# awkrail/svpc

Measured on AMD Instinct MI355X. Metric: train steps/sec (vivt, batch=16, clip_seq=12), higher is better.
Workload: dtype bf16x3; 1 GPU; MODEL_TYPE=vivt train step: N=16 videos/GPU x S=12 clips x Lv=100 frames x F=3072, Lt=22, D=768, H=12, L=6 (enc+step-enc+dec), V=951, A=384, E=10; dropout .1/.1/.4; fwd+bwd+allreduce+clip+BertAdam; mode=bf16x3, global_batch=16, parallelism=dp1, launch=hipGraph replay, gpus_requested=1

## Files before the change

### include/svpc_hip.h

```cpp
#ifndef SVPC_HIP_H
#define SVPC_HIP_H
#include <stddef.h>
#ifdef __cplusplus
extern "C" {
#endif

typedef struct ihipStream_t* svpc_stream_t;
typedef unsigned long long svpc_u64;

#define SVPC_ACT_NONE 0
#define SVPC_ACT_RELU 1
#define SVPC_ACT_GELU 2
#define SVPC_ACT_SIGMOID 3

const char* svpc_last_error(void);
int svpc_abi_version(void);

int svpc_ln_fwd(const float* x, const int* src_rows, const float* res, const float* gamma, const float* beta, float* y,
                float* mean, float* rstd, int R, int D, float eps, float p_pre, unsigned site_pre, float p_post,
                unsigned site_post, const svpc_u64* seed, const float* add1, int mod1, const float* add2, const int* idx2,
                svpc_stream_t stream);
int svpc_ln_fwd_t(const void* x, int x_dt, const int* src_rows, const void* res, const float* gamma, const float* beta, void* y,
                  int y_dt, float* mean, float* rstd, int R, int D, float eps, float p_pre, unsigned site_pre, float p_post,
                  unsigned site_post, const svpc_u64* seed, const float* add1, int mod1, const float* add2, const int* idx2,
// ... 85 lines not shown
} svpc_wgrad_problem;
int svpc_gemm_group_wgrad_max(void);
int svpc_gemm_group_wgrad_bf16_p8_ok(const void* problems, int n);
int svpc_gemm_group_wgrad_bf16_p8(const void* problems, int n, float* workspace, size_t workspace_bytes, svpc_stream_t stream);
int svpc_gemm_group_wgrad_bf16(const svpc_wgrad_problem* problems, int n, svpc_stream_t stream);
int svpc_gemm_group_wgrad_bf16_ws(const svpc_wgrad_problem* problems, int n, float* workspace, size_t workspace_bytes,
                                  svpc_stream_t stream);
int svpc_gemm_group_wgrad(const svpc_wgrad_problem* problems, int n, svpc_stream_t stream);
int svpc_act_bwd(const float* dy, const float* aux, float* dz, size_t n, int act, float p, unsigned site, const svpc_u64* seed,
                 svpc_stream_t stream);

int svpc_act_bwd_t(const void* dy, const void* aux, void* dz, int dt, size_t n, int act, float p, unsigned site, const svpc_u64* seed,
                   svpc_stream_t stream);

int svpc_attn_fwd(const float* Q, int ldq, const float* K, int ldk, const float* V, int ldv, float* O, int ldo, float* LSE,
                  const int* seq, int n_seq, int H, int dh, int max_q, int max_k, const float* key_mask, int causal, float scale,
                  float p_drop, unsigned site, const svpc_u64* seed, svpc_stream_t stream);
int svpc_attn_q1_fwd(const float* Q, int ldq, const float* K, int ldk, const float* V, int ldv, float* O, int ldo, float* LSE,
                     const int* seq, int n_seq, int H, int dh, int max_k, const float* key_mask, float scale, svpc_stream_t stream);
int svpc_attn_q1_ln_supported(int D, int dh, int n_keys, int ldq, int ldkv, int ldnew, int ldx, int ldo);
int svpc_attn_q1_ln_fwd(const float* Q, int ldq, float* K, float* V, int ldkv, int k_stride, int n_keys, const float* newK, const float* newV,
                        int ldnew, const float* X, int ldx, const float* gamma, const float* beta, float eps, float* O, int ldo, int T, int D,
                        int dh, float scale, svpc_stream_t stream);
int svpc_attn_q1_ln_idx_fwd(const float* Q, int ldq, float* K, float* V, int ldkv, int k_stride, int n_keys, const int* key_rows, int ld_rows,
                            int q_group, const float* newK, const float* newV, int ldnew, const float* X, int ldx, const float* gamma,
                            const float* beta, float eps, float* O, int ldo, int T, int D, int dh, float scale, svpc_stream_t stream);
int svpc_attn_bwd(const float* Q, int ldq, const float* K, int ldk, const float* V, int ldv, const float* O, int ldo,
                  const float* LSE, const float* dO, int lddo, float* dQ, int lddq, float* dK, int lddk, float* dV, int lddv,
                  float* delta, const int* seq, int n_seq, int H, int dh, int max_q, int max_k, const float* key_mask, int causal,
                  float scale, float p_drop, unsigned site, const svpc_u64* seed, svpc_stream_t stream);

int svpc_attn_mfma_supported(int dh, int max_q, int max_k, int ldq, int ldk, int ldv, int dt );
int svpc_attn_mfma_fwd(const float* Q, int ldq, const float* K, int ldk, const float* V, int ldv, float* O, int ldo, float* LSE,
                       const int* seq, int n_seq, int H, int dh, int max_q, int max_k, const float* key_mask, int causal,
                       float scale, float p_drop, unsigned site, const svpc_u64* seed, svpc_stream_t stream);
int svpc_attn_mfma_bwd(const float* Q, int ldq, const float* K, int ldk, const float* V, int ldv, const float* O, int ldo,
                       const float* LSE, const float* dO, int lddo, float* dQ, int lddq, float* dK, int lddk, float* dV, int lddv,
                       const int* seq, int n_seq, int H, int dh, int max_q, int max_k, const float* key_mask, int causal, float scale,
                       float p_drop, unsigned site, const svpc_u64* seed, svpc_stream_t stream);

int svpc_attn_mfma_fwd_t(const void* Q, int ldq, const void* K, int ldk, const void* V, int ldv, void* O, int ldo, int dt, float* LSE,
                         const int* seq, int n_seq, int H, int dh, int max_q, int max_k, const float* key_mask, int causal,
                         float scale, float p_drop, unsigned site, const svpc_u64* seed, svpc_stream_t stream);
int svpc_attn_stream_x3_fwd(const void* Q, int ldq, int q_lo, const void* K, int ldk, int k_lo, const void* V, int ldv, int v_lo, void* O,
                            int ldo, int o_lo, float* LSE, const int* seq, int n_seq, int H, int dh, int max_q, int max_k,
                            const float* key_mask, float scale, float p_drop, unsigned site, const svpc_u64* seed, svpc_stream_t stream);
int svpc_attn_q1s_supported(int dh, int max_k, int ldq, int ldk, int ldv, int k_lo, int v_lo);
int svpc_attn_q1s_fwd(const float* Q, int ldq, const void* K, int ldk, int k_lo, const void* V, int ldv, int v_lo, float* O, int ldo, float* LSE,
                      const int* seq, int n_seq, int H, int dh, int max_k, const float* key_mask, float scale, float p_drop, unsigned site,
                      const svpc_u64* seed, svpc_stream_t stream);
int svpc_attn_q1s_bwd(const float* Q, int ldq, const void* K, int ldk, int k_lo, const void* V, int ldv, int v_lo, const float* dO, int lddo,
                      float* dQ, int lddq, void* dK, int lddk, void* dV, int lddv, const int* seq, int n_seq, int H, int dh, int max_k,
                      const float* key_mask, float scale, float p_drop, unsigned site, const svpc_u64* seed, svpc_stream_t stream);
int svpc_attn_x3_fwd(const void* Q, int ldq, int q_lo, const void* K, int ldk, int k_lo, const void* V, int ldv, int v_lo, void* O, int ldo,
                     int o_lo, float* LSE, const int* seq, int n_seq, int H, int dh, int max_q, int max_k, const float* key_mask, int causal,
                     float scale, float p_drop, unsigned site, const svpc_u64* seed, svpc_stream_t stream);
int svpc_attn_pipe_enable(int on);
int svpc_attn_pipe_debug(int bits, void* buf);
int svpc_attn_mfma_bwd_t(const void* Q, int ldq, const void* K, int ldk, const void* V, int ldv, const void* O, int ldo, int dt,
                         const float* LSE, const void* dO, int lddo, void* dQ, int lddq, void* dK, int lddk, void* dV, int lddv,
                         const int* seq, int n_seq, int H, int dh, int max_q, int max_k, const float* key_mask, int causal, float scale,
                         float p_drop, unsigned site, const svpc_u64* seed, svpc_stream_t stream);

int svpc_sim_recur_fwd(const float* q, const float* c, const float* w4f, const float* E0, const int* step_off, const int* step_len,
                       const int* ent_off, const int* ent_len, int n_videos, int e_max, int D, float* e_out, float* ebar,
                       float* eall, svpc_stream_t stream);
int svpc_sim_recur_bwd(const float* q, const float* c, const float* w4f, const float* E0, const int* step_off, const int* step_len,
                       const int* ent_off, const int* ent_len, int n_videos, int e_max, int D, const float* e_out,
                       const float* ebar, const float* eall, const float* de, const float* debar, const float* deall, float* dq,
                       float* dc, float* dw4f, float* dE0, svpc_stream_t stream);

int svpc_sim_heads_groups(int T);
int svpc_sim_heads_fwd(const float* hh, const float* fb, const float* W3, const float* b3, const float* W4, const float* b4, float* c, float* w,
                       int T, int D, int Wd, svpc_stream_t stream);
int svpc_sim_heads_bwd(const float* hh, const float* fb, const float* W3, const float* W4, const float* c, const float* dc, const float* dw,
                       float* dhh, float* dfb, float* part3, float* part4, int T, int D, int Wd, svpc_stream_t stream);

int svpc_cross_attn_ln_supported(int D, int H, int lt, int nm);
int svpc_cross_attn_ln_fwd(const void* q, int q_dt, int ldq, int loq, const void* x1, int x_dt, int ldx, int lox, const void* k, const void* v,
                           int kv_dt, int ld_kv, int lokv, const float* gamma, const float* beta, float eps, void* y, int y_dt, int ldy, int loy,
                           float* probs, float* mean, float* rstd, int T, int lt, int nm, int D, int H, float scale, float p_drop, unsigned site,
                           const svpc_u64* seed, svpc_stream_t stream);
int svpc_cross_attn_ln_bwd(const void* q, int q_dt, int ldq, int loq, const void* x1, int x_dt, int ldx, int lox, const void* k, const void* v,
                           int kv_dt, int ld_kv, int lokv, const float* gamma, const float* probs, const float* mean, const float* rstd,
                           const void* dy, int dy_dt, int lddy, void* dq, void* dres, int dg_dt, int lddg, void* dk, void* dv, int dkv_dt,
                           int ld_dkv, float* part_ln, int T, int lt, int nm, int D, int H, float scale, float p_drop, unsigned site,
                           const svpc_u64* seed, svpc_stream_t stream);
int svpc_cross_attn_ln_fwd_r(const void* q, int q_dt, int ldq, int loq, const void* x1, int x_dt, int ldx, int lox, const void* k, const void* v,
                             int kv_dt, int ld_kv, int lokv, const float* gamma, const float* beta, float eps, void* y, int y_dt, int ldy, int loy,
                             float* probs, float* mean, float* rstd, int T, int lt, int nm, int D, int H, float scale, float p_drop, unsigned site,
                             const svpc_u64* seed, const int* row_off, const int* row_len, svpc_stream_t stream);
int svpc_cross_attn_ln_bwd_r(const void* q, int q_dt, int ldq, int loq, const void* x1, int x_dt, int ldx, int lox, const void* k, const void* v,
                             int kv_dt, int ld_kv, int lokv, const float* gamma, const float* probs, const float* mean, const float* rstd,
                             const void* dy, int dy_dt, int lddy, void* dq, void* dres, int dg_dt, int lddg, void* dk, void* dv, int dkv_dt,
                             int ld_dkv, float* part_ln, int T, int lt, int nm, int D, int H, float scale, float p_drop, unsigned site,
                             const svpc_u64* seed, const int* row_off, const int* row_len, svpc_stream_t stream);

int svpc_ptr_attn_fwd(const float* dec, const float* proj, const float* bank, const int* step_ne, float* pi, float* att, int T,
                      int lt, int e_max, int D, svpc_stream_t stream);
int svpc_ptr_attn_pgen_fwd(const float* dec, const float* proj, const float* bank, const int* step_ne, float* pi, float* att,
                           const float* pgen_w, const float* pgen_b, float* pgen, int T, int lt, int e_max, int D, svpc_stream_t stream);
int svpc_ptr_attn_bwd(const float* dec, const float* proj, const float* bank, const int* step_ne, const float* pi, const float* dpi,
                      const float* datt, float* ddec, float* dproj, float* dbank, int T, int lt, int e_max, int D,
                      svpc_stream_t stream);
int svpc_ptr_attn_gate_fwd(const float* dec, const float* proj, const float* bank, const int* step_ne, float* pi, const float* pgen_w,
                           const float* pgen_b, float* pgen, int T, int lt, int e_max, int D, svpc_stream_t stream);
// ... 223 lines not shown
```

### svpc_amd/grad_tail.py

```python
from __future__ import annotations

import ctypes
import os

import torch

from . import _lib

USE_GROUPED_WGRAD = os.environ.get("SVPC_NO_GROUPED_WGRAD", "") == ""
GROUP_BF16 = os.environ.get("SVPC_NO_GROUP_BF16", "") == ""
GROUP_FLUSH_AT = int(os.environ.get("SVPC_GROUP_FLUSH_AT", "16"))
GROUP_MAX_TILES = int(os.environ.get("SVPC_GROUP_MAX_TILES", "1200"))
COLSUM_FLUSH_AT = 48

_WQ16 = []
_WQ = []
_CQ = []
_FQ = []
_JOIN_QUEUED = [False]
GRAD_READY_HOOK = None
HOOKS_PAUSED = [0]
_OPS = []


# ... 71 lines not shown
    rows, n_out = dz.shape
    n_in = x.shape[1]
    if rows < 1 or n_out % 4 or n_in % 4 or dz.stride(0) % 4 or x.stride(0) % 4 or wgrad.stride(0) % 4:
        return False
    if (dz.data_ptr() | x.data_ptr()) % 16 or dz.stride(1) != 1 or x.stride(1) != 1 or not wgrad.is_contiguous():
        return False
    tiles = -(-n_out // 64) * -(-n_in // 64)
    if tiles > GROUP_MAX_TILES:
        return False
    wp = wgrad.data_ptr()
    if any(q[2].data_ptr() == wp for q in _WQ):
        flush_wgrads(bf16=False)
    _WQ.append((dz, x, wgrad, bgrad))
    if len(_WQ) >= min(GROUP_FLUSH_AT, _lib.load().svpc_gemm_group_wgrad_max()):
        flush_wgrads(bf16=False)
    _queue_end_of_backward_join()
    return True


def _problem_table(queue):
    probs = (_WgradProblem * len(queue))()
    for i, (dz, x, wg, bg) in enumerate(queue):
        probs[i] = _WgradProblem(dz.data_ptr(), x.data_ptr(), wg.data_ptr(), bg.data_ptr() if bg is not None else None, dz.shape[1],
                                 x.shape[1], dz.shape[0], dz.stride(0), x.stride(0), wg.stride(0))
    return probs


def flush_wgrads(bf16=True):
    o = _ops()
    if _WQ16 and bf16:
        probs = _problem_table(_WQ16)
        ws = o._ws(_WQ16[0][0].device)
        p8w = o.USE_P8W and _lib.load().svpc_gemm_group_wgrad_bf16_p8_ok(ctypes.addressof(probs), len(_WQ16)) == 1
        done = list(_WQ16)
        del _WQ16[:]
        if not p8w:
            for i, (dz, x, wg, bg) in enumerate(done):
                if bg is not None:
                    probs[i].db = None
                    defer_colsum(dz, bg)
        _lib.call("gemm_group_wgrad_bf16_p8" if p8w else "gemm_group_wgrad_bf16_ws", ctypes.addressof(probs), len(done),
                  ws.data_ptr(), ws.numel() * 4, o._stream())
        for _, _, wg, bg in done:
            _ready(wg, "w")
            if bg is not None and p8w:
                _ready(bg, "b")
    if not _WQ:
        return
    probs = _problem_table(_WQ)
    _lib.call("gemm_group_wgrad", ctypes.addressof(probs), len(_WQ), o._stream())
    done = list(_WQ)
    del _WQ[:]
    for _, _, wg, bg in done:
        _ready(wg, "w")
        if bg is not None:
            _ready(bg, "b")


def defer_finalize(partial, groups, ncols, out0, out1=None, split=None):
    tgt = (out0.data_ptr(), out1.data_ptr() if out1 is not None else 0)
    if any(q[1].data_ptr() in tgt or (q[2] is not None and q[2].data_ptr() in tgt) for q in _FQ):
        flush_finalizes()
    _FQ.append((partial, out0, out1, int(groups), int(ncols), int(ncols if split is None else split)))
    if len(_FQ) >= _lib.load().svpc_multi_finalize_max():
        flush_finalizes()
    _queue_end_of_backward_join()


def defer_colsum(x, out):
    R, C = x.shape
    chunks = _lib.load().svpc_colsum_chunks(R)
    partial = torch.empty(chunks * C, dtype=torch.float32, device=x.device)
    if len(_CQ) >= COLSUM_FLUSH_AT:
        flush_finalizes()
    _CQ.append((x, partial))
    defer_finalize(partial, chunks, C, out)


def _flush_colsums():
    if not _CQ:
        return
    o = _ops()
    ents = (_ColsumEntry * len(_CQ))()
    for i, (x, partial) in enumerate(_CQ):
        ents[i] = _ColsumEntry(x.data_ptr(), partial.data_ptr(), o._dt(x), x.stride(0), x.shape[0], x.shape[1])
    _lib.call("multi_colsum", ctypes.addressof(ents), len(_CQ), o._stream())
    del _CQ[:]


def flush_finalizes():
    _flush_colsums()
    if not _FQ:
        return
    ents = (_FinalizeEntry * len(_FQ))()
    for i, (partial, o0, o1, g, nc, sp) in enumerate(_FQ):
        ents[i] = _FinalizeEntry(partial.data_ptr(), o0.data_ptr(), (o1 if o1 is not None else o0).data_ptr(), g, nc, sp)
    _lib.call("multi_finalize", ctypes.addressof(ents), len(_FQ), _ops()._stream())
    done = list(_FQ)
    del _FQ[:]
    for _, o0, o1, _, _, _ in done:
        _ready(o0, "b" if o1 is None else None)
        if o1 is not None:
            _ready(o1)


def bias_grad(dz, target):
    M, N = dz.shape
# ... 30 lines not shown
```

### svpc_amd/model.py

```python
from __future__ import annotations

import math

import numpy as np
import torch
import torch.nn as nn

from . import ops
from .ops_common import ACT_GELU, ACT_NONE, ACT_RELU, ACT_SIGMOID, BulkUpload, FIdx, Idx

PAD_ROW = 0


def _sinusoid(max_len, d):
    pe = torch.zeros(max_len, d)
    pos = torch.arange(0, max_len).float().unsqueeze(1)
    div = torch.exp(torch.arange(0, d, 2).float() * -(math.log(10000.0) / d))
    pe[:, 0::2] = torch.sin(pos * div)
    pe[:, 1::2] = torch.cos(pos * div)
    return pe


def _i32(v, device):
    return torch.tensor(v, dtype=torch.int32, device=device)
# ... 110 lines not shown

class BertOutput(nn.Module):
    def __init__(self, config):
        super().__init__()
        self.dense = nn.Linear(config.intermediate_size, config.hidden_size)
        self.LayerNorm = BertLayerNorm(config.hidden_size, eps=config.layer_norm_eps)


class _Ctx:

    def __init__(self, config, training, rng):
        self.H = config.num_attention_heads
        self.eps = config.layer_norm_eps
        self.training = training
        self.rng = rng
        self.p_h = config.hidden_dropout_prob
        self.p_a = config.attention_probs_dropout_prob

    def drop(self, p):
        if not self.training or p <= 0.0:
            return None
        return (p, self.rng, self.rng.site())


class BertLayerNoMemoryUntied(nn.Module):

    def __init__(self, config):
        super().__init__()
        self.attention = BertAttention(config)
        self.hidden_intermediate = BertIntermediate(config)
        self.memory_intermediate = BertIntermediate(config)
        self.output = BertOutput(config)

    def run(self, h, seq, key_mask, cx):
        D = h.shape[1]
        w, b, wg, bg, w16 = self.attention.self.packed()
        qkv = ops.linear(h, w, b, wgrad=wg, bgrad=bg, w16=w16)
        ctx = ops.attention(qkv, qkv, (0, D, 2 * D), D, cx.H, seq, key_mask=key_mask, causal=False, drop=cx.drop(cx.p_a))
        so = self.attention.output
        ao = ops.linear(ctx, so.dense.weight, so.dense.bias)
        x1 = ops.layernorm(ao, so.LayerNorm.weight, so.LayerNorm.bias, cx.eps, residual=h, pre_drop=cx.drop(cx.p_h), sink=True)
        it = ops.linear(x1, self.hidden_intermediate.dense.weight, self.hidden_intermediate.dense.bias, act=ACT_GELU, fuse_act_bwd=True)
        o = ops.linear(it, self.output.dense.weight, self.output.dense.bias)
        return ops.layernorm(o, self.output.LayerNorm.weight, self.output.LayerNorm.bias, cx.eps,
                             residual=x1, pre_drop=cx.drop(cx.p_h), sink=True)


    def run_rows(self, h, sel_rows, seq_sel, key_mask, cx):
        D = h.shape[1]
        att = self.attention.self
        hq, h = ops.take_rows_f32_alias(h, sel_rows)
        q = ops.linear(hq, att.query.weight, att.query.bias)
        wkv, bkv, wg, bg, w16 = att.packed("kv")
        kv = ops.linear(h, wkv, bkv, wgrad=wg, bgrad=bg, w16=w16)
        ctx = ops.attention(q, kv, (0, 0, D), D, cx.H, seq_sel, key_mask=key_mask, causal=False, drop=cx.drop(cx.p_a)).float()
        so = self.attention.output
        ao = ops.linear(ctx, so.dense.weight, so.dense.bias)
        x1 = ops.layernorm(ao, so.LayerNorm.weight, so.LayerNorm.bias, cx.eps, residual=hq, pre_drop=cx.drop(cx.p_h))
        it = ops.linear(x1, self.hidden_intermediate.dense.weight, self.hidden_intermediate.dense.bias, act=ACT_GELU)
        o = ops.linear(it, self.output.dense.weight, self.output.dense.bias)
        return ops.layernorm(o, self.output.LayerNorm.weight, self.output.LayerNorm.bias, cx.eps,
                             residual=x1, pre_drop=cx.drop(cx.p_h))


class BertEncoderNoMemoryUntied(nn.Module):

    def __init__(self, config):
        super().__init__()
        self.config = config
        self.layer = nn.ModuleList([BertLayerNoMemoryUntied(config) for _ in range(config.num_hidden_layers)])

    def run(self, h, seq, key_mask, cx, last_rows=None, last_seq=None):
        n = len(self.layer)
        for i, layer in enumerate(self.layer):
            if last_rows is not None and i == n - 1:
                h = layer.run_rows(h, last_rows, last_seq, key_mask, cx)
            else:
                h = layer.run(h, seq, key_mask, cx)
        return h

    def forward(self, hidden_states, attention_mask, diagonal_mask=False, output_all_encoded_layers=True):
        B, L, D = hidden_states.shape
        cx = _Ctx(self.config, self.training, ops.default_rng(hidden_states.device))
        seq = ops.SeqInfo.uniform(B, L, L, hidden_states.device)
        km = attention_mask.reshape(-1).float().contiguous()
        h = self.run(hidden_states.reshape(B * L, D).contiguous(), seq, km, cx)
        return [h.view(B, L, D)]


class BertDecoderLayerNoMemoryUntied(nn.Module):

    def __init__(self, config):
        super().__init__()
        self.self_attention = BertSelfAttention(config)
        self.norm1 = BertLayerNorm(config.hidden_size, eps=config.layer_norm_eps)
        self.dec_enc_attention = BertSelfAttention(config)
        self.norm2 = BertLayerNorm(config.hidden_size, eps=config.layer_norm_eps)
        self.output = BertOutput(config)

    def run(self, x, text_mask, mem, seq_self, seq_cross, mem_mask, cx, kvc=None):
        D = x.shape[1]
        w, b, wg, bg, w16 = self.self_attention.packed()
        qkv = ops.linear(x, w, b, wgrad=wg, bgrad=bg, w16=w16)
        sa = ops.attention(qkv, qkv, (0, D, 2 * D), D, cx.H, seq_self, key_mask=text_mask, causal=True,
                           drop=cx.drop(cx.p_a))
        x1 = ops.layernorm(sa, self.norm1.weight, self.norm1.bias, cx.eps, residual=x, sink=True)
        ca_m = self.dec_enc_attention
        qc = ops.linear(x1, ca_m.query.weight, ca_m.query.bias)
# ... 811 lines not shown
```

### svpc_amd/ops.py

```python
from __future__ import annotations

import ctypes
import math
import numbers
import os
import struct

import torch
from torch.autograd import Function as _TorchFunction

from . import _lib
from .ops_common import ACT_GELU, ACT_NONE, ACT_RELU, ACT_SIGMOID, FIdx, Idx, SeqInfo, as_idx
from .grad_tail import (HOOKS_PAUSED, _WgradProblem, _queue_end_of_backward_join, _ready, bias_grad, defer_colsum,
                        defer_finalize, defer_partials, defer_wgrad, flush_finalizes, flush_pending, flush_wgrads, hooks_paused, join_side)

_WS = {}
_WS_BYTES = 256 << 20


_DEV_IDX = [None]


def _stream():
    i = _DEV_IDX[0]
# ... 920 lines not shown
S4T_MIN_TILES = int(os.environ.get("SVPC_S4T_MIN_TILES", "64"))
S4T_MAX_TILES = int(os.environ.get("SVPC_S4T_MAX_TILES", "640"))
X3_BIG_TILES = int(os.environ.get("SVPC_X3_BIG_TILES", "128"))


def attention(qt, kvt, cols, D, n_heads, seq, key_mask=None, causal=False, drop=None):
    require_split_tag(qt, "attention (queries)")
    require_split_tag(kvt, "attention (keys / values)")
    if qt.dtype == torch.float32 and kvt.dtype == torch.bfloat16 and kvt is not qt:
        dh = D // n_heads
        lo = lo_off(kvt) or 0
        if (USE_Q1S and _fast() and seq.max_q == 1 and not causal and qt.is_cuda and qt.stride(1) == 1 and kvt.stride(1) == 1 and
                (qt.data_ptr() | kvt.data_ptr()) % 16 == 0 and
                _lib.load().svpc_attn_q1s_supported(dh, seq.max_k, qt.stride(0), kvt.stride(0), kvt.stride(0), lo, lo) == 1):
            return _Attention.apply(qt, kvt, cols, D, n_heads, seq, key_mask, causal, drop)
        if lo_off(kvt) is not None:
            kvt = to_f32(kvt)
        else:
            qt = qt.to(torch.bfloat16)
    split = lo_off(qt) is not None or lo_off(kvt) is not None
    if ABLATE is not None and split and kvt is qt and ABLATE.get("attn"):
        flags = ABLATE["attn"] if seq.max_q > 32 else ""
        if flags:
            assert not torch.is_grad_enabled()
            c = new_split(qt.shape[0], qt.shape[1], qt.device)
            c.copy_(qt.detach()); _lo_view(c).copy_(_lo_view(qt))
            lo = _lo_view(c)
            if "q" in flags:
                lo[:, cols[0]:cols[0] + D].zero_()
            if "k" in flags:
                lo[:, cols[1]:cols[1] + D].zero_()
            if "v" in flags:
                lo[:, cols[2]:cols[2] + D].zero_()
            qt = kvt = c
    if split:
        dh = D // n_heads
        ok = ((not causal or (seq.max_q <= 32 and seq.max_k <= 32)) and lo_off(qt) is not None and lo_off(kvt) is not None and
              _lib.load().svpc_attn_mfma_supported(dh, seq.max_q, seq.max_k, 8, 8, 8, 1) == 1 and qt.stride(0) % 8 == 0 and kvt.stride(0) % 8 == 0 and
              ((qt.data_ptr() + cols[0] * 2) | (kvt.data_ptr() + cols[1] * 2) | (kvt.data_ptr() + cols[2] * 2)) % 16 == 0)
        if not ok:
            same = kvt is qt
            qt = to_f32(qt)
            kvt = qt if same else to_f32(kvt)
            split = False
    if kvt.requires_grad and torch.is_grad_enabled() and seq.shares_keys:
        raise _lib.SvpcKernelError("attention: sequences that share key / value rows have no backward (every sequence writes its own dK / dV "
                                   "rows: they would be overwritten, not summed) — replicate the rows through a differentiable gather")
    out = _Attention.apply(qt, kvt, cols, D, n_heads, seq, key_mask, causal, drop)
    if split:
        out._svpc_lo = out.shape[1]
    return out


class _SplitCols(Function):

    @staticmethod
    def forward(ctx, wide, n, gbuf):
        w = wide.shape[1] // n
        ctx.gbuf, ctx.n, ctx.w = gbuf, n, w
        return tuple(wide[:, i * w:(i + 1) * w] for i in range(n))

    @staticmethod
    def backward(ctx, *grads):
        g, w = ctx.gbuf, ctx.w
        for i, gi in enumerate(grads):
            blk = g[:, i * w:(i + 1) * w]
            if gi is None:
                blk.zero_()
            elif gi.data_ptr() != blk.data_ptr() or gi.stride() != blk.stride():
                blk.copy_(gi)
        ctx.gbuf = None
        return g, None, None


def attn_q1_ln(q, kv, k_stride, n_keys, residual, gamma, beta, eps, n_heads, new_kv=None, key_rows=None, q_group=1):
    T, D = residual.shape
    indexed = key_rows is not None or q_group != 1
    if key_rows is not None:
        if not (key_rows.dtype == torch.int32 and key_rows.is_contiguous() and key_rows.dim() == 2 and key_rows.shape[0] == T
                and key_rows.shape[1] >= n_keys and key_rows.device == residual.device):
            raise ValueError("attn_q1_ln: key_rows must be a contiguous int32 (T, >= n_keys) table on the rows' device")
    elif q_group != 1 and (q_group < 1 or T % q_group or kv.shape[0] < (T // q_group) * k_stride):
        raise ValueError("attn_q1_ln: q_group must divide T and the kv rows must cover T / q_group sentences")
    if torch.is_grad_enabled() and (q.requires_grad or residual.requires_grad):
        return None
    ts = (q, kv, residual) + ((new_kv,) if new_kv is not None else ())
    if not all(t.is_cuda and t.dtype == torch.float32 and lo_off(t) is None and t.stride(1) == 1 for t in ts) or D % n_heads:
        return None
    lib = _lib.load()
    ldn = new_kv.stride(0) if new_kv is not None else 0
    if lib.svpc_attn_q1_ln_supported(D, D // n_heads, n_keys, q.stride(0), kv.stride(0), ldn, residual.stride(0), D) != 1:
        return None
    if any(t.data_ptr() % 16 for t in ts) or kv.shape[1] != 2 * D or k_stride < n_keys:
        return None
    out = torch.empty(T, D, dtype=torch.float32, device=q.device)
    nk = new_kv.data_ptr() if new_kv is not None else None
    if indexed:
        _lib.call("attn_q1_ln_idx_fwd", _p(q), q.stride(0), kv.data_ptr(), kv.data_ptr() + 4 * D, kv.stride(0), k_stride, n_keys, _p(key_rows),
                  key_rows.shape[1] if key_rows is not None else 0, int(q_group), nk, (nk + 4 * D) if nk is not None else None, ldn,
                  _p(residual), residual.stride(0), _p(gamma), _p(beta), float(eps), _p(out), D, T, D, D // n_heads, 1.0 / math.sqrt(D // n_heads),
                  _stream())
        return out
    _lib.call("attn_q1_ln_fwd", _p(q), q.stride(0), kv.data_ptr(), kv.data_ptr() + 4 * D, kv.stride(0), k_stride, n_keys, nk,
              (nk + 4 * D) if nk is not None else None, ldn, _p(residual), residual.stride(0), _p(gamma), _p(beta), float(eps), _p(out), D, T, D,
              D // n_heads, 1.0 / math.sqrt(D // n_heads), _stream())
    return out
# ... 2207 lines not shown
```

Measured before the change: 90.46 steps/s (one step = 16 clip-sequences per GPU; whole-job aggregate).

## Fold K/V projection into single-query CLS attention via per-head weight expansion

For the selected-row attention, where each clip has one query row, this replaces the full K/V linear over all frame rows plus attention. Instead it multiplies the query into per-head key-weight rows (U = q·Wk_h), scores the raw inputs against U, pools the raw inputs by probability, and contracts with Wv afterwards. The aim is to avoid materialising the K/V projection over every frame row (a large GEMM over roughly 19200+ rows) when there is only one query. The backward mirrors this and adds per-head weight-gradient GEMMs. It adds new kernels with more scalar FMA work and its own dropout and gradient-hook handling.

```diff
diff --git a/include/svpc_hip.h b/include/svpc_hip.h
--- a/include/svpc_hip.h
+++ b/include/svpc_hip.h
@@ -161,6 +161,17 @@
 int svpc_attn_q1s_bwd(const float* Q, int ldq, const void* K, int ldk, int k_lo, const void* V, int ldv, int v_lo, const float* dO, int lddo,
                       float* dQ, int lddq, void* dK, int lddk, void* dV, int lddv, const int* seq, int n_seq, int H, int dh, int max_k,
                       const float* key_mask, float scale, float p_drop, unsigned site, const svpc_u64* seed, svpc_stream_t stream);
+int svpc_cls_fold_supported(int H, int D, int max_k, int x_kind, int ldx, int x_lo);
+int svpc_cls_fold_expand(const float* A, int lda, const float* W, int ldw, const float* bias, float* Out, float* Dot, int n, int H, int D,
+                         svpc_stream_t stream);
+int svpc_cls_fold_contract(const float* W, int ldw, const float* T, const float* bias, const float* Ps, float* Out, int ldo, int n, int H, int D,
+                           const float* bgA, int bg_lda, const float* bgPs, float* bgOut, int bg_accumulate, svpc_stream_t stream);
+int svpc_cls_fold_fwd(const void* X, int x_kind, int ldx, int x_lo, const float* U, float* Pooled, float* Psum, float* P, const int* seq, int n_seq,
+                      int H, int D, int max_k, const float* key_mask, float scale, float p_drop, unsigned site, const svpc_u64* seed,
+                      svpc_stream_t stream);
+int svpc_cls_fold_bwd(const void* X, int x_kind, int ldx, int x_lo, const float* U, const float* dPooled, const float* dPsum, const float* P,
+                      void* dX, int lddx, float* dU, const int* seq, int n_seq, int H, int D, int max_k, float scale, float p_drop, unsigned site,
+                      const svpc_u64* seed, svpc_stream_t stream);
 int svpc_attn_x3_fwd(const void* Q, int ldq, int q_lo, const void* K, int ldk, int k_lo, const void* V, int ldv, int v_lo, void* O, int ldo,
                      int o_lo, float* LSE, const int* seq, int n_seq, int H, int dh, int max_q, int max_k, const float* key_mask, int causal,
                      float scale, float p_drop, unsigned site, const svpc_u64* seed, svpc_stream_t stream);
diff --git a/svpc_amd/csrc/cls_fold.hip b/svpc_amd/csrc/cls_fold.hip
--- /dev/null
+++ b/svpc_amd/csrc/cls_fold.hip
@@ -0,0 +1,432 @@
+#include "common.h"
+
+typedef __bf16 bf16x4 __attribute__((ext_vector_type(4)));
+typedef float cf4 __attribute__((ext_vector_type(4)));
+
+constexpr int CF_HMAX = 16;
+constexpr int CF_KMAX = 128;
+constexpr int CF_NW = 8;
+
+struct ClsFoldArgs {
+    const void* X; int ldx, x_lo;
+    const float* U;
+    const float* G;
+    const float* dPsum;
+    float* Out;
+    float* Psum;
+    float* P;
+    void* dX; int lddx;
+    const int* seq; int n_seq, H, D;
+    const float* key_mask; float scale, p_drop; uint32_t site; const u64* seed;
+};
+
+template <int ST>
+__device__ __forceinline__ cf4 cf_load4(const void* X, size_t row, int ld, int lo, int col) {
+    if (ST == 0) return *reinterpret_cast<const cf4*>(reinterpret_cast<const float*>(X) + row * ld + col);
+    const __bf16* p = reinterpret_cast<const __bf16*>(X) + row * ld + col;
+    const bf16x4 h = *reinterpret_cast<const bf16x4*>(p);
+    cf4 r = {(float)h[0], (float)h[1], (float)h[2], (float)h[3]};
+    if (ST == 2) {
+        const bf16x4 l = *reinterpret_cast<const bf16x4*>(p + lo);
+        r.x += (float)l[0]; r.y += (float)l[1]; r.z += (float)l[2]; r.w += (float)l[3];
+    }
+    return r;
+}
+__device__ __forceinline__ float cf_dot4(cf4 a, cf4 b, float acc) {
+    return fmaf(a.w, b.w, fmaf(a.z, b.z, fmaf(a.y, b.y, fmaf(a.x, b.x, acc))));
+}
+__device__ __forceinline__ void cf_axpy4(float w, cf4 x, cf4& acc) {
+    acc = w * x + acc;
+}
+__device__ __forceinline__ void cf_axpy4s(float w, cf4 x, cf4& acc) {
+    acc.x = fmaf(w, x.x, acc.x); acc.y = fmaf(w, x.y, acc.y); acc.z = fmaf(w, x.z, acc.z); acc.w = fmaf(w, x.w, acc.w);
+}
+
+__device__ __forceinline__ void cf_stage(const float* src, float* dst, int n) {
+    for (int i = 4 * threadIdx.x; i < n; i += 4 * blockDim.x) *reinterpret_cast<cf4*>(dst + i) = *reinterpret_cast<const cf4*>(src + i);
+}
+
+template <int ST, int NHG>
+__device__ __forceinline__ void cf_load_pair(const ClsFoldArgs& a, int k_off, int k_len, int j0, int lane, cf4 (&x)[2][NHG]) {
+    const size_t r0 = (size_t)k_off + min(j0, k_len - 1), r1 = (size_t)k_off + min(j0 + 1, k_len - 1);
+#pragma unroll
+    for (int i = 0; i < NHG; ++i) {
+        const int col = 4 * (lane + 64 * i);
+        const bool live = col < a.D;
+        const cf4 x0 = cf_load4<ST>(a.X, r0, a.ldx, a.x_lo, live ? col : a.D - 4), x1 = cf_load4<ST>(a.X, r1, a.ldx, a.x_lo, live ? col : a.D - 4);
+        x[0][i] = live ? x0 : cf4{0.f, 0.f, 0.f, 0.f};
+        x[1][i] = live ? x1 : cf4{0.f, 0.f, 0.f, 0.f};
+    }
+}
+template <int ST, int NHG>
+__device__ __forceinline__ void cf_rows_dot(const ClsFoldArgs& a, int k_off, int k_len, const float* V, float* S, int wave, int lane) {
+    constexpr int STEP = 2 * CF_NW;
+    cf4 xc[2][NHG], xn[2][NHG], xf[2][NHG];
+#pragma unroll
+    for (int i = 0; i < NHG; ++i) xn[0][i] = xn[1][i] = xf[0][i] = xf[1][i] = cf4{0.f, 0.f, 0.f, 0.f};
+    if (2 * wave < k_len) cf_load_pair<ST, NHG>(a, k_off, k_len, 2 * wave, lane, xn);
+    if (2 * wave + STEP < k_len) cf_load_pair<ST, NHG>(a, k_off, k_len, 2 * wave + STEP, lane, xf);
+#pragma unroll 1
+    for (int j0 = 2 * wave; j0 < k_len; j0 += STEP) {
+#pragma unroll
+        for (int i = 0; i < NHG; ++i) { xc[0][i] = xn[0][i]; xc[1][i] = xn[1][i]; xn[0][i] = xf[0][i]; xn[1][i] = xf[1][i]; }
+        if (j0 + 2 * STEP < k_len) cf_load_pair<ST, NHG>(a, k_off, k_len, j0 + 2 * STEP, lane, xf);
+        float acc[32];
+#pragma unroll
+        for (int i = 0; i < 32; ++i) acc[i] = 0.f;
+#pragma unroll
+        for (int i = 0; i < NHG; ++i) {
+            const int col = min(4 * (lane + 64 * i), a.D - 4);
+#pragma unroll
+            for (int h = 0; h < 4 * NHG; ++h) {
+                const cf4 v = *reinterpret_cast<const cf4*>(V + min(h, a.H - 1) * a.D + col);
+                acc[h] = cf_dot4(v, xc[0][i], acc[h]);
+                acc[CF_HMAX + h] = cf_dot4(v, xc[1][i], acc[CF_HMAX + h]);
+            }
+        }
+        const float s = wave_reduce_scatter32(acc, lane);
+        const int h = (lane >> 1) & (CF_HMAX - 1), j = j0 + (lane >> 5);
+        if (!(lane & 1) && h < a.H && j < k_len) S[h * CF_KMAX + j] = s;
+    }
+}
+
+template <int ST, int NHG>
+__device__ __forceinline__ void cf_rows_wsum(const ClsFoldArgs& a, int c, int k_off, int k_len, const float* W, float* R, int wave, int lane) {
+    constexpr int UN = NHG <= 3 ? 6 : 4, KS = CF_NW / NHG;
+    const int cg = wave % NHG, ks = wave / NHG;
+    const int col = cg * 256 + 4 * lane;
+    const bool live = col < a.D, active = ks < KS;
+    const int colc = live ? col : 0;
+    const int per = (k_len + KS - 1) / KS, jb = ks * per, je = min(jb + per, k_len);
+    cf4 acc[4 * NHG];
+#pragma unroll
+    for (int h = 0; h < 4 * NHG; ++h) acc[h] = cf4{0.f, 0.f, 0.f, 0.f};
+    if (active) {
+#pragma unroll 1
+        for (int j0 = jb; j0 < je; j0 += UN) {
+            cf4 x[UN];
+#pragma unroll
+            for (int u = 0; u < UN; ++u) x[u] = cf_load4<ST>(a.X, (size_t)k_off + min(j0 + u, k_len - 1), a.ldx, a.x_lo, colc);
+#pragma unroll
+            for (int u = 0; u < UN; ++u) {
+                const int j = min(j0 + u, CF_KMAX - 1);
+                const bool in = j0 + u < je;
+#pragma unroll
+                for (int h = 0; h < 4 * NHG; ++h) cf_axpy4s(in ? W[min(h, a.H - 1) * CF_KMAX + j] : 0.f, x[u], acc[h]);
+            }
+        }
+    }
+    __syncthreads();
+#pragma unroll 1
+    for (int r = 0; r < KS; ++r) {
+        if (active && ks == r && live) {
+#pragma unroll
+            for (int h = 0; h < 4 * NHG; ++h) {
+                cf4* p = reinterpret_cast<cf4*>(R + min(h, a.H - 1) * a.D + col);
+                cf4 t = acc[h];
+                if (r > 0) t += *p;
+                if (h < a.H) *p = t;
+            }
+        }
+        __syncthreads();
+    }
+    cf_stage(R, a.Out + (size_t)c * a.H * a.D, a.H * a.D);
+}
+
+
+template <int ST, int NHG>
+__global__ __launch_bounds__(CF_NW * 64) void cls_fold_fwd_kernel(ClsFoldArgs a) {
+    extern __shared__ __align__(16) float cf_lds[];
+    float* U = cf_lds;
+    float* S = cf_lds + a.H * a.D;
+    const int c = blockIdx.x, lane = threadIdx.x & 63, wave = __builtin_amdgcn_readfirstlane(threadIdx.x >> 6);
+    const int k_off = a.seq[2 * a.n_seq + c], k_len = a.seq[3 * a.n_seq + c];
+    cf_stage(a.U + (size_t)c * a.H * a.D, U, a.H * a.D);
+    __syncthreads();
+    cf_rows_dot<ST, NHG>(a, k_off, k_len, U, S, wave, lane);
+    __syncthreads();
+    const u64 seed = a.p_drop > 0.f ? a.seed[0] : 0ull;
+    const float inv_keep = 1.0f / (1.0f - a.p_drop);
+#pragma unroll 1
+    for (int h = wave; h < a.H; h += CF_NW) {
+        float sc[2], p[2];
+#pragma unroll
+        for (int kk = 0; kk < 2; ++kk) {
+            const int k = lane + 64 * kk;
+            sc[kk] = k < k_len ? S[h * CF_KMAX + k] * a.scale + (1.0f - (a.key_mask ? a.key_mask[k_off + k] : 1.0f)) * -10000.0f : -INFINITY;
+        }
+        const float mx = wave_max(fmaxf(sc[0], sc[1]));
+        p[0] = sc[0] > -INFINITY ? expf(sc[0] - mx) : 0.f;
+        p[1] = sc[1] > -INFINITY ? expf(sc[1] - mx) : 0.f;
+        const float inv = 1.0f / wave_sum(p[0] + p[1]);
+        const u64 row = (u64)c * a.H + h;
+        float ps = 0.f;
+#pragma unroll
+        for (int kk = 0; kk < 2; ++kk) {
+            const int k = lane + 64 * kk;
+            p[kk] *= inv;
+            a.P[row * CF_KMAX + k] = p[kk];
+            const float m = a.p_drop > 0.f ? attn_drop_scale(seed, a.site, row, (uint32_t)k, a.p_drop, inv_keep) : 1.0f;
+            const float pt = p[kk] * m;
+            S[h * CF_KMAX + k] = pt;
+            ps += pt;
+        }
+        ps = wave_sum(ps);
+        if (lane == 0) a.Psum[row] = ps;
+    }
+    __syncthreads();
+    cf_rows_wsum<ST, NHG>(a, c, k_off, k_len, S, U, wave, lane);
+}
+
+template <int ST, int NHG>
+__global__ __launch_bounds__(CF_NW * 64) void cls_fold_bwd_kernel(ClsFoldArgs a) {
+    extern __shared__ __align__(16) float cf_lds[];
+    float* U = cf_lds;
+    float* G = U + a.H * a.D;
+    float* DS = G + a.H * a.D;
+    float* PT = DS + a.H * CF_KMAX;
+    const int c = blockIdx.x, lane = threadIdx.x & 63, wave = __builtin_amdgcn_readfirstlane(threadIdx.x >> 6);
+    const int k_off = a.seq[2 * a.n_seq + c], k_len = a.seq[3 * a.n_seq + c];
+    cf_stage(a.U + (size_t)c * a.H * a.D, U, a.H * a.D);
+    cf_stage(a.G + (size_t)c * a.H * a.D, G, a.H * a.D);
+    __syncthreads();
+    cf_rows_dot<ST, NHG>(a, k_off, k_len, G, DS, wave, lane);
+    __syncthreads();
+    const u64 seed = a.p_drop > 0.f ? a.seed[0] : 0ull;
+    const float inv_keep = 1.0f / (1.0f - a.p_drop);
+#pragma unroll 1
+    for (int h = wave; h < a.H; h += CF_NW) {
+        const u64 row = (u64)c * a.H + h;
+        const float dps = a.dPsum[row];
+        float p[2], m[2], dp[2];
+#pragma unroll
+        for (int kk = 0; kk < 2; ++kk) {
+            const int k = lane + 64 * kk;
+            p[kk] = a.P[row * CF_KMAX + k];
+            m[kk] = a.p_drop > 0.f ? attn_drop_scale(seed, a.site, row, (uint32_t)k, a.p_drop, inv_keep) : 1.0f;
+            dp[kk] = k < k_len ? m[kk] * (DS[h * CF_KMAX + k] + dps) : 0.f;
+        }
+        const float delta = wave_sum(p[0] * dp[0] + p[1] * dp[1]);
+#pragma unroll
+        for (int kk = 0; kk < 2; ++kk) {
+            const int k = lane + 64 * kk;
+            DS[h * CF_KMAX + k] = p[kk] * (dp[kk] - delta) * a.scale;
+            PT[h * CF_KMAX + k] = p[kk] * m[kk];
+        }
+    }
+    __syncthreads();
+    if (a.dX) {
+        const int nch = a.D >> 2;
+#pragma unroll 1
+        for (int j0 = 2 * wave; j0 < k_len; j0 += 2 * CF_NW) {
+            const int j1 = min(j0 + 1, k_len - 1);
+#pragma unroll 1
+            for (int ch = lane; ch < nch; ch += 64) {
+                cf4 d0 = cf4{0.f, 0.f, 0.f, 0.f}, d1 = d0;
+#pragma unroll 1
+                for (int h = 0; h < a.H; ++h) {
+                    const cf4 u = *reinterpret_cast<const cf4*>(U + h * a.D + 4 * ch), g = *reinterpret_cast<const cf4*>(G + h * a.D + 4 * ch);
+                    cf_axpy4(DS[h * CF_KMAX + j0], u, d0); cf_axpy4(PT[h * CF_KMAX + j0], g, d0);
+                    cf_axpy4(DS[h * CF_KMAX + j1], u, d1); cf_axpy4(PT[h * CF_KMAX + j1], g, d1);
+                }
+                if (ST == 0) {
+                    float* o = reinterpret_cast<float*>(a.dX) + 4 * ch;
+                    *reinterpret_cast<cf4*>(o + (size_t)(k_off + j0) * a.lddx) = d0;
+                    if (j1 != j0) *reinterpret_cast<cf4*>(o + (size_t)(k_off + j1) * a.lddx) = d1;
+                } else {
+                    __bf16* o = reinterpret_cast<__bf16*>(a.dX) + 4 * ch;
+                    bf16x4 b0, b1;
+                    b0[0] = (__bf16)d0.x; b0[1] = (__bf16)d0.y; b0[2] = (__bf16)d0.z; b0[3] = (__bf16)d0.w;
+                    b1[0] = (__bf16)d1.x; b1[1] = (__bf16)d1.y; b1[2] = (__bf16)d1.z; b1[3] = (__bf16)d1.w;
+                    *reinterpret_cast<bf16x4*>(o + (size_t)(k_off + j0) * a.lddx) = b0;
+                    if (j1 != j0) *reinterpret_cast<bf16x4*>(o + (size_t)(k_off + j1) * a.lddx) = b1;
+                }
+            }
+        }
+    }
+    cf_rows_wsum<ST, NHG>(a, c, k_off, k_len, DS, U, wave, lane);
+}
+
+__global__ __launch_bounds__(256) void cls_fold_expand_kernel(const float* __restrict__ A, int lda, const float* __restrict__ W, int ldw,
+                                                               const float* __restrict__ bias, float* __restrict__ Out, float* __restrict__ Dot,
+                                                               int n, int H, int D) {
+    __shared__ __align__(16) float As[16][64];
+    const int h = blockIdx.y, c0 = blockIdx.z * 16, t = threadIdx.x;
+#pragma unroll
+    for (int i = 0; i < 4; ++i) {
+        const int idx = t + 256 * i, cc = idx >> 6, d = idx & 63;
+        As[cc][d] = c0 + cc < n ? A[(size_t)(c0 + cc) * lda + 64 * h + d] : 0.f;
+    }
+    __syncthreads();
+    const int j = blockIdx.x * 256 + t;
+    if (j < D) {
+        float acc[16];
+#pragma unroll
+        for (int cc = 0; cc < 16; ++cc) acc[cc] = 0.f;
+        const float* wp = W + (size_t)(64 * h) * ldw + j;
+#pragma unroll 2
+        for (int d = 0; d < 64; d += 4) {
+            const float w0 = wp[(size_t)d * ldw], w1 = wp[(size_t)(d + 1) * ldw], w2 = wp[(size_t)(d + 2) * ldw], w3 = wp[(size_t)(d + 3) * ldw];
+#pragma unroll
+            for (int cc = 0; cc < 16; ++cc) {
+                const cf4 q = *reinterpret_cast<const cf4*>(&As[cc][d]);
+                acc[cc] = fmaf(q.w, w3, fmaf(q.z, w2, fmaf(q.y, w1, fmaf(q.x, w0, acc[cc]))));
+            }
+        }
+#pragma unroll
+        for (int cc = 0; cc < 16; ++cc)
+            if (c0 + cc < n) Out[((size_t)(c0 + cc) * H + h) * D + j] = acc[cc];
+    }
+    if (Dot != nullptr && blockIdx.x == 0 && t < 16 && c0 + t < n) {
+        float s = 0.f;
+        for (int d = 0; d < 64; ++d) s = fmaf(As[t][d], bias[64 * h + d], s);
+        Dot[(size_t)(c0 + t) * H + h] = s;
+    }
+}
+
+constexpr int CF_CT = 8;
+template <int NHG>
+__global__ __launch_bounds__(256) void cls_fold_contract_kernel(const float* __restrict__ W, int ldw, const float* __restrict__ T,
+                                                                 const float* __restrict__ bias, const float* __restrict__ Ps,
+                                                                 float* __restrict__ Out, int ldo, int n, int H, int D,
+                                                                 const float* __restrict__ bgA, int bg_lda, const float* __restrict__ bgPs,
+                                                                 float* __restrict__ bgOut, int bg_accumulate) {
+    extern __shared__ __align__(16) float cf_lds[];
+    const int h = blockIdx.x, c0 = blockIdx.y * CF_CT, lane = threadIdx.x & 63, wave = __builtin_amdgcn_readfirstlane(threadIdx.x >> 6);
+    if (c0 >= n) {
+        float s = 0.f;
+#pragma unroll 8
+        for (int c = wave; c < n; c += 4) s = fmaf(bgA[(size_t)c * bg_lda + 64 * h + lane], bgPs[(size_t)c * H + h], s);
+        cf_lds[64 * wave + lane] = s;
+        __syncthreads();
+        if (wave == 0) {
+            const float t = (cf_lds[lane] + cf_lds[64 + lane]) + (cf_lds[128 + lane] + cf_lds[192 + lane]);
+            bgOut[64 * h + lane] = bg_accumulate ? bgOut[64 * h + lane] + t : t;
+        }
+        return;
+    }
+    for (int i = 4 * threadIdx.x; i < CF_CT * D; i += 4 * 256) {
+        const int cc = i / D, j = i - cc * D;
+        *reinterpret_cast<cf4*>(cf_lds + i) =
+            c0 + cc < n ? *reinterpret_cast<const cf4*>(T + ((size_t)(c0 + cc) * H + h) * D + j) : cf4{0.f, 0.f, 0.f, 0.f};
+    }
+    __syncthreads();
+#pragma unroll 2
+    for (int d0 = 16 * wave; d0 < 16 * wave + 16; d0 += 4) {
+        cf4 w[4][NHG];
+#pragma unroll
+        for (int i = 0; i < NHG; ++i) {
+            const int col = 4 * (lane + 64 * i);
+            const bool live = col < D;
+#pragma unroll
+            for (int r = 0; r < 4; ++r) {
+                const cf4 t = *reinterpret_cast<const cf4*>(W + (size_t)(64 * h + d0 + r) * ldw + (live ? col : D - 4));
+                w[r][i] = live ? t : cf4{0.f, 0.f, 0.f, 0.f};
+            }
+        }
+        float acc[32];
+#pragma unroll
+        for (int i = 0; i < 32; ++i) acc[i] = 0.f;
+#pragma unroll
+        for (int i = 0; i < NHG; ++i) {
+            const int col = min(4 * (lane + 64 * i), D - 4);
+#pragma unroll
+            for (int cc = 0; cc < CF_CT; ++cc) {
+                const cf4 tv = *reinterpret_cast<const cf4*>(cf_lds + cc * D + col);
+#pragma unroll
+                for (int r = 0; r < 4; ++r) acc[r * CF_CT + cc] = cf_dot4(w[r][i], tv, acc[r * CF_CT + cc]);
+            }
+        }
+        float s = wave_reduce_scatter32(acc, lane);
+        const int r = lane >> 4, cc = (lane >> 1) & (CF_CT - 1), row = 64 * h + d0 + r;
+        if (!(lane & 1) && c0 + cc < n) {
+            if (bias != nullptr) s = fmaf(bias[row], Ps[(size_t)(c0 + cc) * H + h], s);
+            Out[(size_t)(c0 + cc) * ldo + row] = s;
+        }
+    }
+}
+
+static bool cf_shape_ok(int H, int D, int max_k) { return H >= 1 && H <= CF_HMAX && D == 64 * H && max_k >= 1 && max_k <= CF_KMAX; }
+static bool cf_stream_ok(const void* X, int kind, int ldx, int x_lo) {
+    return kind >= 0 && kind <= 2 && ldx % 8 == 0 && x_lo % 8 == 0 && (kind == 2) == (x_lo != 0) && (((uintptr_t)X) & 15) == 0;
+}
+
+template <int ST, int NHG>
+static int cf_launch_rows(bool bwd, const ClsFoldArgs& a, hipStream_t stream) {
+    const size_t lds = ((bwd ? 2 : 1) * (size_t)a.H * a.D + (bwd ? 2 : 1) * (size_t)a.H * CF_KMAX) * sizeof(float);
+    const void* fn = bwd ? reinterpret_cast<const void*>(&cls_fold_bwd_kernel<ST, NHG>) : reinterpret_cast<const void*>(&cls_fold_fwd_kernel<ST, NHG>);
+    if (lds > 64 * 1024) { const int rc = svpc_raise_lds_once(fn, "cls_fold"); if (rc) return rc; }
+    if (bwd) hipLaunchKernelGGL((cls_fold_bwd_kernel<ST, NHG>), dim3(a.n_seq), dim3(CF_NW * 64), lds, stream, a);
+    else hipLaunchKernelGGL((cls_fold_fwd_kernel<ST, NHG>), dim3(a.n_seq), dim3(CF_NW * 64), lds, stream, a);
+    return svpc_check_launch(bwd ? "cls_fold_bwd" : "cls_fold_fwd");
+}
+template <int ST>
+static int cf_launch_rows(bool bwd, const ClsFoldArgs& a, hipStream_t stream) {
+    const int nhg = (a.H + 3) / 4;
+    return nhg == 1 ? cf_launch_rows<ST, 1>(bwd, a, stream) : nhg == 2 ? cf_launch_rows<ST, 2>(bwd, a, stream)
+         : nhg == 3 ? cf_launch_rows<ST, 3>(bwd, a, stream) : cf_launch_rows<ST, 4>(bwd, a, stream);
+}
+static int cf_launch_rows(bool bwd, int kind, const ClsFoldArgs& a, hipStream_t stream) {
+    return kind == 0 ? cf_launch_rows<0>(bwd, a, stream) : kind == 1 ? cf_launch_rows<1>(bwd, a, stream) : cf_launch_rows<2>(bwd, a, stream);
+}
+
+extern "C" {
+
+int svpc_cls_fold_supported(int H, int D, int max_k, int x_kind, int ldx, int x_lo) {
+    return cf_shape_ok(H, D, max_k) && cf_stream_ok(nullptr, x_kind, ldx, x_lo) ? 1 : 0;
+}
+
+int svpc_cls_fold_expand(const float* A, int lda, const float* W, int ldw, const float* bias, float* Out, float* Dot, int n, int H, int D,
+                         hipStream_t stream) {
+    if (n == 0) return 0;
+    SVPC_REQUIRE(cf_shape_ok(H, D, 1) && (Dot == nullptr) == (bias == nullptr), "cls_fold_expand: unsupported shape");
+    hipLaunchKernelGGL(cls_fold_expand_kernel, dim3(ceil_div(D, 256), H, ceil_div(n, 16)), dim3(256), 0, stream, A, lda, W, ldw, bias, Out, Dot, n, H, D);
+    return svpc_check_launch("cls_fold_expand");
+}
+
+int svpc_cls_fold_contract(const float* W, int ldw, const float* T, const float* bias, const float* Ps, float* Out, int ldo, int n, int H, int D,
+                           const float* bgA, int bg_lda, const float* bgPs, float* bgOut, int bg_accumulate, hipStream_t stream) {
+    if (n == 0) return 0;
+    SVPC_REQUIRE(cf_shape_ok(H, D, 1) && ldw % 4 == 0 && ((((uintptr_t)W) | ((uintptr_t)T)) & 15) == 0 && (Ps == nullptr) == (bias == nullptr) &&
+                     ((bgA == nullptr) == (bgPs == nullptr)) && ((bgA == nullptr) == (bgOut == nullptr)),
+                 "cls_fold_contract: unsupported shape / alignment");
+    const dim3 grid(H, ceil_div(n, CF_CT) + (bgA != nullptr ? 1 : 0)), block(256);
+    const size_t lds = (size_t)CF_CT * D * sizeof(float);
+#define CF_CONTRACT(NHG) hipLaunchKernelGGL(cls_fold_contract_kernel<NHG>, grid, block, lds, stream, W, ldw, T, bias, Ps, Out, ldo, n, H, D, bgA, bg_lda, \
+                                            bgPs, bgOut, bg_accumulate)
+    switch ((H + 3) / 4) {
+        case 1: CF_CONTRACT(1); break;
+        case 2: CF_CONTRACT(2); break;
+        case 3: CF_CONTRACT(3); break;
+        default: CF_CONTRACT(4); break;
+    }
+#undef CF_CONTRACT
+    return svpc_check_launch("cls_fold_contract");
+}
+
+int svpc_cls_fold_fwd(const void* X, int x_kind, int ldx, int x_lo, const float* U, float* Pooled, float* Psum, float* P, const int* seq, int n_seq,
+                      int H, int D, int max_k, const float* key_mask, float scale, float p_drop, unsigned site, const u64* seed,
+                      hipStream_t stream) {
+    if (n_seq == 0) return 0;
+    SVPC_REQUIRE(cf_shape_ok(H, D, max_k) && cf_stream_ok(X, x_kind, ldx, x_lo), "cls_fold_fwd: unsupported shape / alignment");
+    SVPC_REQUIRE(p_drop <= 0.f || seed != nullptr, "cls_fold_fwd: dropout needs a seed pointer");
+    ClsFoldArgs a{};
+    a.X = X; a.ldx = ldx; a.x_lo = x_lo; a.U = U; a.Out = Pooled; a.Psum = Psum; a.P = P; a.seq = seq; a.n_seq = n_seq; a.H = H; a.D = D;
+    a.key_mask = key_mask; a.scale = scale; a.p_drop = p_drop; a.site = site; a.seed = seed;
+    return cf_launch_rows(false, x_kind, a, stream);
+}
+
+int svpc_cls_fold_bwd(const void* X, int x_kind, int ldx, int x_lo, const float* U, const float* dPooled, const float* dPsum, const float* P,
+                      void* dX, int lddx, float* dU, const int* seq, int n_seq, int H, int D, int max_k, float scale, float p_drop, unsigned site,
+                      const u64* seed, hipStream_t stream) {
+    if (n_seq == 0) return 0;
+    SVPC_REQUIRE(cf_shape_ok(H, D, max_k) && cf_stream_ok(X, x_kind, ldx, x_lo) && lddx % 4 == 0 && (((uintptr_t)dX) & 15) == 0,
+                 "cls_fold_bwd: unsupported shape / alignment");
+    SVPC_REQUIRE(p_drop <= 0.f || seed != nullptr, "cls_fold_bwd: dropout needs a seed pointer");
+    ClsFoldArgs a{};
+    a.X = X; a.ldx = ldx; a.x_lo = x_lo; a.U = U; a.G = dPooled; a.dPsum = dPsum; a.Out = dU; a.P = const_cast<float*>(P); a.dX = dX; a.lddx = lddx; a.seq = seq;
+    a.n_seq = n_seq; a.H = H; a.D = D; a.scale = scale; a.p_drop = p_drop; a.site = site; a.seed = seed;
+    return cf_launch_rows(true, x_kind, a, stream);
+}
+
+}
diff --git a/svpc_amd/grad_tail.py b/svpc_amd/grad_tail.py
--- a/svpc_amd/grad_tail.py
+++ b/svpc_amd/grad_tail.py
@@ -147,7 +147,7 @@
     done = list(_WQ)
     del _WQ[:]
     for _, _, wg, bg in done:
-        _ready(wg, "w")
+        _ready(getattr(wg, "_svpc_ready_as", wg), "w")
         if bg is not None:
             _ready(bg, "b")
 
diff --git a/svpc_amd/model.py b/svpc_amd/model.py
--- a/svpc_amd/model.py
+++ b/svpc_amd/model.py
@@ -186,8 +186,12 @@
         hq, h = ops.take_rows_f32_alias(h, sel_rows)
         q = ops.linear(hq, att.query.weight, att.query.bias)
         wkv, bkv, wg, bg, w16 = att.packed("kv")
-        kv = ops.linear(h, wkv, bkv, wgrad=wg, bgrad=bg, w16=w16)
-        ctx = ops.attention(q, kv, (0, 0, D), D, cx.H, seq_sel, key_mask=key_mask, causal=False, drop=cx.drop(cx.p_a)).float()
+        fold = getattr(ops, "cls_fold_selected", None)
+        if fold is not None and fold(h, seq_sel, D, cx.H):
+            ctx = ops.cls_fold(q, h, wkv, bkv, cx.H, seq_sel, key_mask=key_mask, drop=cx.drop(cx.p_a), wgrad=wg, bgrad=bg)
+        else:
+            kv = ops.linear(h, wkv, bkv, wgrad=wg, bgrad=bg, w16=w16)
+            ctx = ops.attention(q, kv, (0, 0, D), D, cx.H, seq_sel, key_mask=key_mask, causal=False, drop=cx.drop(cx.p_a)).float()
         so = self.attention.output
         ao = ops.linear(ctx, so.dense.weight, so.dense.bias)
         x1 = ops.layernorm(ao, so.LayerNorm.weight, so.LayerNorm.bias, cx.eps, residual=hq, pre_drop=cx.drop(cx.p_h))
diff --git a/svpc_amd/ops.py b/svpc_amd/ops.py
--- a/svpc_amd/ops.py
+++ b/svpc_amd/ops.py
@@ -996,6 +996,103 @@
     return out
 
 
+_CLS_FOLD_ENV = os.environ.get("SVPC_CLS_FOLD", "")
+CLS_FOLD = None if _CLS_FOLD_ENV == "" else _CLS_FOLD_ENV != "0"
+CLS_FOLD_MIN_ROWS = int(os.environ.get("SVPC_CLS_FOLD_MIN_ROWS", "19200"))
+
+
+def cls_fold_selected(x, seq, D, n_heads):
+    if CLS_FOLD is False or not torch.is_grad_enabled():
+        return False
+    if CLS_FOLD is None and x.shape[0] < CLS_FOLD_MIN_ROWS:
+        return False
+    ok = (x.dim() == 2 and x.shape[1] == D and D == 64 * n_heads and seq.max_q == 1 and min(seq.h_k_len) >= 1 and x.is_cuda and
+          x.stride(1) == 1 and x.dtype in (torch.float32, torch.bfloat16) and x.data_ptr() % 16 == 0 and
+          _lib.load().svpc_cls_fold_supported(n_heads, D, seq.max_k, _kind(x), x.stride(0), lo_off(x) or 0) == 1)
+    if not ok and CLS_FOLD:
+        raise _lib.SvpcKernelError("cls_fold: forced on, but the folded kernels do not take this shape / storage (head dim 64, ≤ 16 heads, "
+                                   "≤ 128 keys per clip, fp32 / bf16 / split rows)")
+    return ok
+
+
+class _ClsFold(Function):
+    @staticmethod
+    def forward(ctx, q, x, w, b, H, seq, key_mask, drop, wgrad, bgrad, x_lo):
+        _need_gpu(q)
+        q, w, b = _c(q), _c(w), _c(b)
+        n, D = q.shape
+        dev = q.device
+        p, site, seed = _drop_args(drop)
+        tbl = seq.table if seq.table.device == dev else seq.table.to(dev)
+        kind = 2 if x_lo is not None else _dt(x)
+        st = _stream()
+        u = torch.empty(n, H, D, dtype=torch.float32, device=dev)
+        _lib.call("cls_fold_expand", _p(q), D, _p(w), D, None, _p(u), None, n, H, D, st)
+        pooled = torch.empty(n, H, D, dtype=torch.float32, device=dev)
+        psum = torch.empty(n, H, dtype=torch.float32, device=dev)
+        prob = torch.empty(n, H, 128, dtype=torch.float32, device=dev)
+        scale = 1.0 / math.sqrt(D // H)
+        _lib.call("cls_fold_fwd", _p(x), kind, x.stride(0), x_lo or 0, _p(u), _p(pooled), _p(psum), _p(prob), _p(tbl), n, H, D, seq.max_k,
+                  _p(key_mask), scale, p, site, _p(seed), st)
+        out = torch.empty(n, D, dtype=torch.float32, device=dev)
+        _lib.call("cls_fold_contract", w.data_ptr() + D * D * 4, D, _p(pooled), b.data_ptr() + D * 4, _p(psum), _p(out), D, n, H, D,
+                  None, 0, None, None, 0, st)
+        ctx.save_for_backward(q, x, w, b, u, pooled, psum, prob, seed, tbl)
+        ctx.cfg = (H, kind, x_lo or 0, seq.max_k, scale, p, site, sum(seq.h_k_len) == x.shape[0])
+        ctx.direct = (wgrad, bgrad)
+        return out
+
+    @staticmethod
+    def backward(ctx, dctx):
+        q, x, w, b, u, pooled, psum, prob, seed, tbl = ctx.saved_tensors
+        H, kind, x_lo, max_k, scale, p, site, covered = ctx.cfg
+        wgrad, bgrad = ctx.direct
+        n, D = q.shape
+        dev = q.device
+        dctx = _c(dctx)
+        st = _stream()
+        wv, bv = w.data_ptr() + D * D * 4, b.data_ptr() + D * 4
+        dpooled = torch.empty(n, H, D, dtype=torch.float32, device=dev)
+        dpsum = torch.empty(n, H, dtype=torch.float32, device=dev)
+        _lib.call("cls_fold_expand", _p(dctx), D, wv, D, bv, _p(dpooled), _p(dpsum), n, H, D, st)
+        du = torch.empty(n, H, D, dtype=torch.float32, device=dev)
+        dx = None
+        if ctx.needs_input_grad[1]:
+            dx = (torch.empty if covered else torch.zeros)(x.shape, dtype=x.dtype, device=dev)
+        _lib.call("cls_fold_bwd", _p(x), kind, x.stride(0), x_lo, _p(u), _p(dpooled), _p(dpsum), _p(prob), _p(dx), D, _p(du), _p(tbl), n, H, D,
+                  max_k, scale, p, site, _p(seed), st)
+        db = bgrad if bgrad is not None else torch.zeros_like(b)
+        dq = torch.empty(n, D, dtype=torch.float32, device=dev)
+        _lib.call("cls_fold_contract", _p(w), D, _p(du), None, None, _p(dq), D, n, H, D, _p(dctx), D, _p(psum), db.data_ptr() + D * 4, 1, st)
+        if bgrad is not None:
+            _ready(bgrad, "b")
+        dw = wgrad if wgrad is not None else torch.zeros_like(w)
+        direct = False
+        for base, dz, xs in ((0, q, du), (D, dctx, pooled)):
+            for h in range(H):
+                dz_h, x_h, dw_h = dz[:, 64 * h:64 * h + 64], xs[:, h], dw[base + 64 * h:base + 64 * h + 64]
+                if wgrad is not None and base == D and h == H - 1:
+                    dw_h._svpc_ready_as = wgrad
+                if not defer_wgrad(dz_h, x_h, dw_h, None):
+                    _gemm(dz_h, dz_h.stride(0), 0, x_h, x_h.stride(0), 0, dw_h, 64, D, n, accumulate=1)
+                    direct = True
+        if wgrad is None:
+            flush_wgrads(bf16=False)
+        elif direct:
+            flush_wgrads(bf16=False)
+            _ready(wgrad, "w")
+        return (dq, dx, None if wgrad is not None else dw, None if bgrad is not None else db, None, None, None, None, None, None, None)
+
+
+def cls_fold(q, x, w, b, n_heads, seq, key_mask=None, drop=None, wgrad=None, bgrad=None):
+    require_split_tag(x, "cls_fold")
+    if wgrad is None:
+        wgrad = _direct(w)
+    if bgrad is None:
+        bgrad = _direct(b)
+    return _ClsFold.apply(q, x, w, b, n_heads, seq, key_mask, drop, wgrad, bgrad, lo_off(x))
+
+
 class _SplitCols(Function):
 
     @staticmethod
```

Result: no change. 90.91 steps/s (one step = 16 clip-sequences per GPU; whole-job aggregate), median of 6 (+0.5%).
